# facebookresearch/goliath

Measured on AMD Instinct MI355X. Metric: relit views/sec (fwd+bwd) at 2048x1334, 250k Gaussians, higher is better.
Workload: dtype f32; 1 GPU; rgca_config2_envrelight; gaussians=250000, views_per_gpu=8, micro_batches=2, world_size=1, dist_backend=none, rccl_world_size=0, parallelism=view-parallel x1, launch=hip_graph_replay

## Files before the change

### goliath_amd/csrc/raster.hip

```cpp
#include <cstdlib>

#include "gol_raster.h"

namespace {

template <bool EXTRA, bool LAZY, int PPL>
__global__ __launch_bounds__(64 * Pix<PPL>::kWaves) void raster_fwd_kernel(
    int N, int img_h, int img_w, int planar, int tiles_x, int tiles_y, const int2* __restrict__ tile_bins,
    const int32_t* __restrict__ sorted_ids, int64_t capacity, const float* __restrict__ records,
    const float* __restrict__ background, float* __restrict__ out_img,
    float* __restrict__ out_extra, float* __restrict__ final_Ts, int32_t* __restrict__ final_idx,
    float* __restrict__ out_alpha, float* __restrict__ out_extra_norm, float norm_lo,
    const float* __restrict__ l1_target, const float* __restrict__ l1_mask, int l1_mask_c,
    uint8_t* __restrict__ l1_sign, float* __restrict__ l1_partial, int n_views) {
  typedef typename Pix<PPL>::fv fv;
  typedef typename Pix<PPL>::iv iv;
  constexpr int NW = Pix<PPL>::kWaves, NT = 64 * NW;
  __shared__ float s_l1[NW];
  __shared__ float4 s_a[kBatch];
  __shared__ float4 s_b[kBatch];
  __shared__ float2 s_c[kBatch];
  __shared__ int32_t s_mask[kBatch];
  const int T = tiles_x * tiles_y;
  const int view = blockIdx.x % n_views, slot = blockIdx.x / n_views;
  const TileCoord tc = tile_of_block(slot, T, tiles_x);
  if (!tc.ok) return;
  const int tid = threadIdx.x, lane = tid & 63, wave = tid >> 6;
  int j, i0;
  lane_pixel<PPL>(tc.tx, tc.ty, wave, lane, j, i0);
  bool in[PPL];
  fv py, live;
#pragma unroll
  for (int q = 0; q < PPL; ++q) {
    in[q] = (i0 + q < img_h) && (j < img_w);
    py[q] = (float)(i0 + q) + 0.5f;
    live[q] = in[q] ? 1.f : 0.f;
  }
  const float px = (float)j + 0.5f;

  const int2 range = tile_bins[(size_t)view * T + tc.tile];
  const int32_t* ids = sorted_ids + (size_t)view * capacity;
  const size_t goff = (size_t)view * N;

  fv T_cur = 1.f;
  iv cur_idx = 0;
  fv acc0 = 0.f, acc1 = 0.f, acc2 = 0.f, acc3 = 0.f;

  const int n_batches = (range.y - range.x + kBatch - 1) / kBatch;
  for (int bb = 0; bb < n_batches; ++bb) {
    if (__syncthreads_and(!any_live<fv, PPL>(live))) break;
    const int batch_start = range.x + bb * kBatch;
    for (int k = tid; k < kBatch; k += NT) {
      const int idx = batch_start + k;
      if (idx < range.y) {
        const Staged st = stage_entry<PPL>(records, goff + (size_t)ids[idx], (float)(tc.tx * 16), (float)(tc.ty * 16));
        s_a[k] = st.a; s_b[k] = st.b; s_c[k] = st.c; s_mask[k] = st.mask;
      } else {
        s_mask[k] = 0;
      }
    }
    __syncthreads();
    const int batch_size = min(kBatch, range.y - batch_start);
    for (int chunk = 0; chunk < batch_size; chunk += 64) {
      unsigned long long bits = gol_ballot((s_mask[chunk + lane] >> wave) & 1);
      if (LAZY && gol_ballot(any_live<fv, PPL>(live)) == 0ull) break;
      while (bits) {
        if (!LAZY && gol_ballot(any_live<fv, PPL>(live)) == 0ull) { chunk = batch_size; break; }
        const int t = chunk + __builtin_ctzll(bits);
        bits &= bits - 1;
        const float4 a4 = s_a[t];
        const float4 b4 = s_b[t];
        const float2 c2 = s_c[t];
        const float dx = a4.x - px;
        const fv dy = a4.y - py;
        fv sigma, e, alpha, vis, next_T;
        visit_falloff<PPL>(a4.z, a4.w, b4.x, dx, dy, sigma, e);
#pragma unroll
        for (int q = 0; q < PPL; ++q) alpha[q] = fminf(GOL_ALPHA_CAP_FWD, b4.y * e[q]);
        bool take[PPL];
        unsigned long long stop_m[PPL];
        const unsigned long long any_stop = fwd_step<PPL>(sigma, alpha, live, T_cur, vis, next_T, take, stop_m);
        bool half_done = false;
        if (!LAZY || any_stop != 0ull) {
#pragma unroll
          for (int q = 0; q < PPL; ++q) {
            const bool stop = __builtin_amdgcn_inverse_ballot_w64(stop_m[q]);
            live[q] = stop ? 0.f : live[q];
            if (LAZY) cur_idx[q] = stop ? (batch_start + t - 1) : cur_idx[q];
          }
          if (LAZY) half_done = gol_ballot(any_live<fv, PPL>(live)) == 0ull;
        }
        fwd_take<PPL>(take, next_T, vis, T_cur);
        acc0 += b4.z * vis; acc1 += b4.w * vis; acc2 += c2.x * vis;
        if (EXTRA) acc3 += c2.y * vis;
        if (!LAZY) {
#pragma unroll
          for (int q = 0; q < PPL; ++q) cur_idx[q] = take[q] ? (batch_start + t) : cur_idx[q];
        }
        if (LAZY && half_done) { chunk = batch_size; break; }
      }
    }
  }
  if (LAZY) {
#pragma unroll
    for (int q = 0; q < PPL; ++q) cur_idx[q] = live[q] != 0.f ? range.y - 1 : cur_idx[q];
  }

  const unsigned hw = (unsigned)img_h * (unsigned)img_w;
  const size_t vplane = (size_t)view * hw;
  float* __restrict__ o_T = final_Ts + vplane;
  int32_t* __restrict__ o_idx = final_idx + vplane;
  float* __restrict__ o_img = out_img + 3 * vplane;
  float* __restrict__ o_ex = (EXTRA && out_extra) ? out_extra + vplane : nullptr;
  float* __restrict__ o_alpha = out_alpha ? out_alpha + vplane : nullptr;
  float* __restrict__ o_norm = (EXTRA && out_extra_norm) ? out_extra_norm + vplane : nullptr;
  const float* __restrict__ i_tgt = l1_target ? l1_target + 3 * vplane : nullptr;
  const float* __restrict__ i_mask = l1_mask ? l1_mask + (size_t)l1_mask_c * vplane : nullptr;
  uint8_t* __restrict__ o_sign = l1_target ? l1_sign + vplane : nullptr;
  const float bg0 = background[0], bg1 = background[1], bg2 = background[2];
  float* __restrict__ o_img1 = o_img + (planar ? hw : 1u);
  float* __restrict__ o_img2 = o_img + (planar ? 2u * hw : 2u);
  const bool bwd_state = range.y > range.x;
  float l1_acc = 0.f;
#pragma unroll
  for (int q = 0; q < PPL; ++q) {
    if (!in[q]) continue;
    const unsigned pix = (unsigned)(i0 + q) * (unsigned)img_w + (unsigned)j;
    const unsigned b4 = pix * 4u;
    const unsigned bimg = planar ? b4 : 3u * b4;
    const float Tq = T_cur[q];
    const float c0 = acc0[q] + Tq * bg0, c1 = acc1[q] + Tq * bg1, c2 = acc2[q] + Tq * bg2, ex = acc3[q];
    *gol_at(o_T, b4) = Tq;
    if (bwd_state || !LAZY) *gol_at(o_idx, b4) = cur_idx[q];
    *gol_at(o_img, bimg) = c0; *gol_at(o_img1, bimg) = c1; *gol_at(o_img2, bimg) = c2;
    if (o_ex) *gol_at(o_ex, b4) = ex;
    if (o_alpha) *gol_at(o_alpha, b4) = 1.f - Tq;
    if (o_norm) *gol_at(o_norm, b4) = ex / fminf(fmaxf(1.f - Tq, norm_lo), 1.f);
    if (i_tgt) {
      const float m0 = i_mask ? *gol_at(i_mask, b4) : 1.f;
      const float cs[3] = {c0, c1, c2};
      unsigned code = 0u;
#pragma unroll
      for (int c = 0; c < 3; ++c) {
        const float m = (i_mask && l1_mask_c == 3) ? *gol_at(i_mask + (size_t)c * hw, b4) : m0;
        const float d = (cs[c] - *gol_at(i_tgt + (size_t)c * hw, b4)) * m;
        l1_acc += fabsf(d);
        code |= (d > 0.f ? 2u : (d < 0.f ? 0u : 1u)) << (2 * c);
      }
      if (bwd_state) *gol_at(o_sign, pix) = (uint8_t)code;
    }
  }
  if (l1_target) {
    const float ws = gol_wave_sum_to_lane63(l1_acc);
    if (lane == 63) s_l1[wave] = ws;
    __syncthreads();
    if (tid == 0) {
      float tot = 0.f;
#pragma unroll
      for (int w = 0; w < NW; ++w) tot += s_l1[w];
      l1_partial[(size_t)view * T + tc.tile] = tot;
    }
  }
}

__global__ __launch_bounds__(1024) void l1_sum_kernel(int n, const float* __restrict__ l1_partial, float scale,
                                                      float* __restrict__ l1_out) {
  __shared__ float s_w[16];
  float a0 = 0.f, a1 = 0.f, a2 = 0.f, a3 = 0.f;
  const int n4 = n >> 2;
  const float4* p4 = reinterpret_cast<const float4*>(l1_partial);
  int i = threadIdx.x;
  for (; i + 3 * 1024 < n4; i += 4 * 1024) {
    const float4 v0 = p4[i], v1 = p4[i + 1024], v2 = p4[i + 2048], v3 = p4[i + 3072];
    a0 += (v0.x + v0.y) + (v0.z + v0.w); a1 += (v1.x + v1.y) + (v1.z + v1.w);
    a2 += (v2.x + v2.y) + (v2.z + v2.w); a3 += (v3.x + v3.y) + (v3.z + v3.w);
  }
  for (; i < n4; i += 1024) { const float4 v = p4[i]; a0 += (v.x + v.y) + (v.z + v.w); }
  if ((int)threadIdx.x < (n & 3)) a1 += l1_partial[4 * n4 + threadIdx.x];
  const float ws = gol_wave_sum_to_lane63((a0 + a1) + (a2 + a3));
  if ((threadIdx.x & 63) == 63) s_w[threadIdx.x >> 6] = ws;
  __syncthreads();
  if (threadIdx.x == 0) {
    float tot = 0.f;
#pragma unroll
    for (int w = 0; w < 16; ++w) tot += s_w[w];
    l1_out[0] = tot * scale;
  }
}

constexpr int kBatchB = 64;
constexpr int kAcc = 12;

static_assert(kBatchB == 64, "raster_bwd_kernel ballots one 64-entry chunk per batch");

template <bool EXTRA, bool PACKED, int PPL>
__global__ __launch_bounds__(64 * Pix<PPL>::kWaves) void raster_bwd_kernel(
    int N, int img_h, int img_w, int planar, int tiles_x, int tiles_y, const int2* __restrict__ tile_bins,
    const int32_t* __restrict__ sorted_ids, int64_t capacity, const float* __restrict__ records,
    const float* __restrict__ background,
    const float* __restrict__ final_Ts, const int32_t* __restrict__ final_idx,
    const float* __restrict__ v_out_img, const float* __restrict__ v_out_extra,
    const float* __restrict__ v_out_alpha, float* __restrict__ v_xy, float* __restrict__ v_conic,
    float* __restrict__ v_colors, float* __restrict__ v_extra, float* __restrict__ v_opacity,
    const uint8_t* __restrict__ v_sign, const float* __restrict__ v_sign_mask, int v_sign_mask_c,
    const float* __restrict__ v_img_scale, float v_img_scale_mul, int n_views) {
  typedef typename Pix<PPL>::fv fv;
  typedef typename Pix<PPL>::iv iv;
  constexpr int NW = Pix<PPL>::kWaves, NT = 64 * NW;
  __shared__ StagedRow s_e[kBatchB];
  __shared__ int32_t s_mask[kBatchB];
  __shared__ int32_t s_id[kBatchB];
  __shared__ __attribute__((aligned(16))) float s_acc[NW][kBatchB][kAcc];
  __shared__ int32_t s_touched[NW][kBatchB];
  __shared__ int32_t s_wmax[NW];
  const int T = tiles_x * tiles_y;
  const int view = blockIdx.x % n_views, slot = blockIdx.x / n_views;
  const TileCoord tc = tile_of_block(slot, T, tiles_x);
  if (!tc.ok) return;
  const int2 range = tile_bins[(size_t)view * T + tc.tile];
  if (range.y <= range.x) return;
  const int tid = threadIdx.x, lane = tid & 63, wave = tid >> 6;
  int j, i0;
  lane_pixel<PPL>(tc.tx, tc.ty, wave, lane, j, i0);
  const float px = (float)j + 0.5f;
  const size_t hw = (size_t)img_h * img_w;
  const int32_t* ids = sorted_ids + (size_t)view * capacity;
  const size_t goff = (size_t)view * N;
  bool in[PPL];
  size_t pp[PPL];
  fv py, T_final;
  iv bin_final;
#pragma unroll
  for (int q = 0; q < PPL; ++q) {
    in[q] = (i0 + q < img_h) && (j < img_w);
    py[q] = (float)(i0 + q) + 0.5f;
    pp[q] = in[q] ? ((size_t)view * img_h + i0 + q) * img_w + j : 0;
    T_final[q] = in[q] ? final_Ts[pp[q]] : 1.f;
    bin_final[q] = in[q] ? final_idx[pp[q]] : (range.x - 1);
  }
  fv T_cur = T_final;
  fv vo0 = 0.f, vo1 = 0.f, vo2 = 0.f, vo3 = 0.f, voa = 0.f;
  {
    const float vsc = (v_img_scale ? v_img_scale[0] : 1.f) * v_img_scale_mul;
    const size_t os = planar ? hw : 1;
#pragma unroll
    for (int q = 0; q < PPL; ++q) {
      if (!in[q]) continue;
      const size_t p = pp[q];
      const int i = i0 + q;
      const size_t o = planar ? (size_t)view * 3 * hw + (size_t)i * img_w + j : 3 * p;
      float g0 = 0.f, g1 = 0.f, g2 = 0.f;
      if (v_out_img) { g0 = v_out_img[o]; g1 = v_out_img[o + os]; g2 = v_out_img[o + 2 * os]; }
      if (v_sign) {
        const unsigned code = v_sign[p];
        float m0 = vsc, m1 = vsc, m2 = vsc;
        if (v_sign_mask) {
          const float* mk = v_sign_mask + (size_t)view * v_sign_mask_c * hw + (size_t)i * img_w + j;
          m0 *= mk[0]; m1 *= (v_sign_mask_c == 3) ? mk[hw] : mk[0]; m2 *= (v_sign_mask_c == 3) ? mk[2 * hw] : mk[0];
        }
        g0 += (float)((int)(code & 3u) - 1) * m0;
        g1 += (float)((int)((code >> 2) & 3u) - 1) * m1;
        g2 += (float)((int)((code >> 4) & 3u) - 1) * m2;
      }
      vo0[q] = g0; vo1[q] = g1; vo2[q] = g2;
      if (EXTRA && v_out_extra) vo3[q] = v_out_extra[p];
      if (v_out_alpha) voa[q] = v_out_alpha[p];
    }
  }
  const fv tail = T_final * (voa - (background[0] * vo0 + background[1] * vo1 + background[2] * vo2));
  fv qsum = 0.f;

  const int wmax = wave_last_entry<PPL>(bin_final);
  if (lane == 0) s_wmax[wave] = wmax;
  __syncthreads();
  int bmax = s_wmax[0];
#pragma unroll
  for (int w = 1; w < NW; ++w) bmax = max(bmax, s_wmax[w]);
  bmax = min(bmax, range.y - 1);
  if (bmax < range.x) return;

  float* acc_lane = &s_acc[wave][0][lane >> 4];
  const int n_batches = (bmax - range.x + kBatchB) / kBatchB;
  auto entry_id = [&](int bb2) {
    const int e = bmax - bb2 * kBatchB - tid;
    return (tid < kBatchB && e >= range.x) ? ids[e] : 0;
  };
  int gid_next = entry_id(0);
  for (int bb = 0; bb < n_batches; ++bb) {
    __syncthreads();
    const int batch_end = bmax - bb * kBatchB;
    const int batch_size = min(kBatchB, batch_end + 1 - range.x);
    const int gid = gid_next;
    if (tid < kBatchB) {
      if (tid < batch_size) {
        const Staged st = stage_entry<PPL>(records, goff + (size_t)gid, (float)(tc.tx * 16), (float)(tc.ty * 16));
        s_e[tid].a = st.a; s_e[tid].b = st.b; s_e[tid].c = st.c; s_mask[tid] = st.mask;
        s_id[tid] = gid;
      } else {
        s_mask[tid] = 0;
      }
    }
    if (bb + 1 < n_batches) gid_next = entry_id(bb + 1);
    (&s_touched[0][0])[tid] = 0;
    __syncthreads();

    const int t0 = max(0, batch_end - wmax);
    unsigned long long bits = gol_ballot((s_mask[lane] >> wave) & 1);
    if (t0 > 0) bits &= ~0ull << t0;
    while (bits) {
      const int t = __builtin_ctzll(bits);
      bits &= bits - 1;
      const float4 a4 = s_e[t].a;
      const float4 b4 = s_e[t].b;
      const float2 c2 = s_e[t].c;
      const int li = batch_end - t;
      const float dx = a4.x - px;
      const fv dy = a4.y - py;
      fv sigma, vis, alpha, ra, fac;
      visit_falloff<PPL>(a4.z, a4.w, b4.x, dx, dy, sigma, vis);
      unsigned long long mv[PPL];
      if (bwd_taken<PPL>(b4.y, vis, sigma, li, bin_final, alpha, mv) == 0ull) continue;
      bool v[PPL];
      bwd_recur<PPL>(mv, alpha, T_cur, v, ra, fac);
      fv w = b4.z * vo0 + b4.w * vo1 + c2.x * vo2;
      if (EXTRA) w += c2.y * vo3;
      fv gop, gy, gyy;
      bwd_moments<PPL>(vis, w, T_cur, ra, fac, tail, v, dy, qsum, gop, gy, gyy);
      float g0s, g1s, g2s, g3 = 0.f;
      if (PPL == 2) {
        g0s = __builtin_fmaf(fac[0], vo0[0], fac[PPL - 1] * vo0[PPL - 1]);
        g1s = __builtin_fmaf(fac[0], vo1[0], fac[PPL - 1] * vo1[PPL - 1]);
        g2s = __builtin_fmaf(fac[0], vo2[0], fac[PPL - 1] * vo2[PPL - 1]);
        if (EXTRA) g3 = __builtin_fmaf(fac[0], vo3[0], fac[PPL - 1] * vo3[PPL - 1]);
      } else {
        g0s = fac[0] * vo0[0]; g1s = fac[0] * vo1[0]; g2s = fac[0] * vo2[0];
        if (EXTRA) g3 = fac[0] * vo3[0];
      }
      const float m0 = lane_sum<PPL>(gop), my = lane_sum<PPL>(gy), myy = lane_sum<PPL>(gyy);
      const float mx = m0 * dx, mxx = mx * dx, mxy = my * dx;
      const float r0 = gol_wave_sum4(g0s, g1s, g2s, m0);
      const float r1 = gol_wave_sum4(mx, my, mxx, mxy);
      const float r2 = gol_wave_sum_to_lane63(myy);
      const float r3 = EXTRA ? gol_wave_sum_to_lane63(g3) : 0.f;
      if ((lane & 15) == 15) {
        float* a = gol_at(acc_lane, (unsigned)t * (unsigned)(kAcc * sizeof(float)));
        a[0] = r0; a[4] = r1;
        if (lane == 63) { a[8 - 3] = r2; a[9 - 3] = r3; }
        s_touched[wave][t] = 1;
      }
    }
    __syncthreads();
    if (PACKED) {
      float* rec = v_colors;
      for (int idx = tid; idx < batch_size * 16; idx += NT) {
        const int t = idx >> 4, c = idx & 15;
        bool any = false;
#pragma unroll
        for (int w = 0; w < NW; ++w) any = any || (s_touched[w][t] != 0);
        if (!any || c > (EXTRA ? 9 : 8)) continue;
        const float4 a4 = s_e[t].a;
        const float4 b4 = s_e[t].b;
        const float nop = -b4.y, cc = b4.x;
        const int k1 = (c == 5) ? 4 : c, k2 = 5;
        const float w1 = (c == 4) ? nop * a4.z * kUnA : (c == 5) ? nop * a4.w * kUnB : (c == 6 || c == 8) ? 0.5f * nop
                       : (c == 7) ? nop : 1.f;
        const float w2 = (c == 4) ? nop * a4.w * kUnB : (c == 5) ? nop * cc * kUnA : 0.f;
        float s1 = 0.f, s2 = 0.f;
#pragma unroll
        for (int w = 0; w < NW; ++w) {
          const bool tw = s_touched[w][t] != 0;
          s1 += tw ? s_acc[w][t][k1] : 0.f;
          s2 += tw ? s_acc[w][t][k2] : 0.f;
        }
        atomicAdd(rec + (goff + (size_t)s_id[t]) * 16 + c, w1 * s1 + w2 * s2);
      }
    } else if (tid < batch_size) {
      float a[kAcc];
#pragma unroll
      for (int k = 0; k < kAcc; ++k) a[k] = 0.f;
      bool any = false;
#pragma unroll
      for (int w = 0; w < NW; ++w) {
        if (s_touched[w][tid]) {
          any = true;
          const float4* q = reinterpret_cast<const float4*>(&s_acc[w][tid][0]);
          const float4 q0 = q[0], q1 = q[1], q2 = q[2];
          a[0] += q0.x; a[1] += q0.y; a[2] += q0.z; a[3] += q0.w;
          a[4] += q1.x; a[5] += q1.y; a[6] += q1.z; a[7] += q1.w;
          a[8] += q2.x; a[9] += q2.y;
        }
      }
      if (any) {
        const size_t g = goff + (size_t)s_id[tid];
        const float4 a4 = s_e[tid].a;
        const float4 b4 = s_e[tid].b;
        const float nop = -b4.y;
        const float3 cn = true_conic(a4.z, a4.w, b4.x);
        atomicAdd(v_colors + 3 * g, a[0]); atomicAdd(v_colors + 3 * g + 1, a[1]); atomicAdd(v_colors + 3 * g + 2, a[2]);
        atomicAdd(v_opacity + g, a[3]);
        atomicAdd(v_xy + 2 * g, nop * (cn.x * a[4] + cn.y * a[5]));
        atomicAdd(v_xy + 2 * g + 1, nop * (cn.y * a[4] + cn.z * a[5]));
        atomicAdd(v_conic + 3 * g, 0.5f * nop * a[6]); atomicAdd(v_conic + 3 * g + 1, nop * a[7]);
        atomicAdd(v_conic + 3 * g + 2, 0.5f * nop * a[8]);
        if (EXTRA && v_extra) atomicAdd(v_extra + g, a[9]);
      }
    }
  }
}

__global__ __launch_bounds__(256) void raster_count_pairs_kernel(int N, int img_h, int img_w, int tiles_x, int tiles_y,
                                                                 const int2* __restrict__ tile_bins,
                                                                 const int32_t* __restrict__ sorted_ids, int64_t capacity,
                                                                 const float* __restrict__ records,
                                                                 const int32_t* __restrict__ final_idx,
                                                                 unsigned long long* __restrict__ counts) {
  __shared__ unsigned long long s_cnt[2];
  const int view = blockIdx.y, tile = blockIdx.x, T = tiles_x * tiles_y;
  const int ty = tile / tiles_x, tx = tile - ty * tiles_x;
  const int j = tx * 16 + (threadIdx.x & 15), i = ty * 16 + (threadIdx.x >> 4);
  if (threadIdx.x < 2) s_cnt[threadIdx.x] = 0ull;
  __syncthreads();
  const int2 range = tile_bins[(size_t)view * T + tile];
  unsigned long long tested = 0, taken = 0;
  if (i < img_h && j < img_w && range.y > range.x) {
    const int last = min(range.y - 1, final_idx[((size_t)view * img_h + i) * img_w + j]);
    const float px = (float)j + 0.5f, py = (float)i + 0.5f;
    for (int li = range.x; li <= last; ++li) {
      const float4* R = reinterpret_cast<const float4*>(records + ((size_t)view * N + sorted_ids[(size_t)view * capacity + li]) * GOL_SPLAT_RECORD);
      const float4 q0 = R[0], q1 = R[1];
      const float dx = q0.x - px, dy = q0.y - py;
      f1 sg, e;
      visit_falloff<1>(q0.z, q0.w, q1.x, dx, f1(dy), sg, e);
      const float alpha = fminf(GOL_ALPHA_CAP_FWD, q1.y * e[0]);
      ++tested;
      taken += (!(sg[0] < 0.f) && !(alpha < GOL_ALPHA_FLOOR)) ? 1 : 0;
    }
  }
  atomicAdd(&s_cnt[0], tested);
  atomicAdd(&s_cnt[1], taken);
  __syncthreads();
  if (threadIdx.x < 2 && s_cnt[threadIdx.x]) atomicAdd(counts + 2 * view + threadIdx.x, s_cnt[threadIdx.x]);
}

__global__ __launch_bounds__(256) void splat_pack_kernel(size_t n, const float* __restrict__ xys,
                                                         const float* __restrict__ conics,
                                                         const float* __restrict__ colors,
                                                         const float* __restrict__ extra,
                                                         const float* __restrict__ opacities,
                                                         float* __restrict__ records) {
  const size_t e = (size_t)blockIdx.x * 256 + threadIdx.x;
  if (e >= n) return;
  gol_record_write(records + e * GOL_SPLAT_RECORD, xys[2 * e], xys[2 * e + 1], conics[3 * e], conics[3 * e + 1],
                   conics[3 * e + 2], opacities[e], colors ? colors[3 * e] : 0.f, colors ? colors[3 * e + 1] : 0.f,
                   colors ? colors[3 * e + 2] : 0.f, extra ? extra[e] : 0.f);
}

}

extern "C" int gol_raster_plan(int B, int* fwd_pixels_per_lane) {
  static const int forced = getenv("GOL_RASTER_PPL") ? atoi(getenv("GOL_RASTER_PPL")) : 0;
  if (fwd_pixels_per_lane) *fwd_pixels_per_lane = (forced == 1 || forced == 2) ? forced : (B <= 2 ? 1 : 2);
  return GOL_OK;
}

extern "C" int gol_raster_count_pairs(int B, int N, int img_h, int img_w, const int32_t* tile_bins, const int32_t* sorted_ids,
                                      int64_t capacity, const float* records, const int32_t* final_idx, uint64_t* counts,
                                      void* stream) {
  GOL_REQUIRE(B >= 0 && N >= 0 && img_h > 0 && img_w > 0, "bad size");
  if (B == 0) return GOL_OK;
  GOL_REQUIRE(tile_bins && final_idx && counts && (capacity == 0 || sorted_ids) && (N == 0 || records), "null pointer");
  hipStream_t s = (hipStream_t)stream;
  if (hipMemsetAsync(counts, 0, sizeof(uint64_t) * 2 * (size_t)B, s) != hipSuccess) {
    gol_set_error("gol_raster_count_pairs: hipMemsetAsync failed");
    return GOL_ERR_LAUNCH;
  }
  const int tiles_x = (img_w + 15) / 16, tiles_y = (img_h + 15) / 16;
  raster_count_pairs_kernel<<<dim3(tiles_x * tiles_y, B), 256, 0, s>>>(
      N, img_h, img_w, tiles_x, tiles_y, reinterpret_cast<const int2*>(tile_bins), sorted_ids, capacity, records, final_idx,
      reinterpret_cast<unsigned long long*>(counts));
  GOL_CHECK_LAUNCH();
  return GOL_OK;
}

extern "C" int gol_splat_pack(int B, int N, const float* xys, const float* conics, const float* colors,
                              const float* extra, const float* opacities, float* records, void* stream) {
  GOL_REQUIRE(B >= 0 && N >= 0, "negative size");
  if (B == 0 || N == 0) return GOL_OK;
  GOL_REQUIRE(xys && conics && opacities && records, "null pointer");
  const size_t n = (size_t)B * N;
  splat_pack_kernel<<<gol_cdiv((long long)n, 256), 256, 0, (hipStream_t)stream>>>(n, xys, conics, colors, extra, opacities,
                                                                                 records);
  GOL_CHECK_LAUNCH();
  return GOL_OK;
}

extern "C" int gol_rasterize_fwd(int B, int N, int img_h, int img_w, int block, int planar, const int32_t* tile_bins,
                                 const int32_t* sorted_ids, int64_t capacity, const float* records, int with_extra,
                                 const float* background, float* out_img,
                                 float* out_extra, float* final_Ts, int32_t* final_idx, float* out_alpha,
                                 float* out_extra_norm, float norm_lo, const float* l1_target, const float* l1_mask,
                                 int l1_mask_c, uint8_t* l1_sign, float* l1_partial, float* l1_out, float l1_scale,
                                 int pixels_per_lane, void* stream) {
  GOL_RASTER_CHECK_DIMS(12, "image too large (32-bit byte offsets inside a view)");
  if (B == 0) return GOL_OK;
  GOL_REQUIRE(tile_bins && background && out_img && final_Ts && final_idx, "null pointer");
  GOL_REQUIRE(capacity == 0 || sorted_ids, "null sorted_ids");
  GOL_REQUIRE(N == 0 || records, "null Gaussian records");
  GOL_REQUIRE((!out_extra && !out_extra_norm) || with_extra || N == 0, "out_extra / out_extra_norm need the extra channel");
  GOL_REQUIRE(!with_extra || out_extra || out_extra_norm, "extra without an output for it");
  GOL_REQUIRE(!l1_target || (planar && l1_sign && l1_partial), "the fused L1 needs planar images, l1_sign and l1_partial");
  GOL_REQUIRE(!l1_mask || (l1_target && (l1_mask_c == 1 || l1_mask_c == 3)), "l1_mask: 1 or 3 channels, with l1_target");
  GOL_REQUIRE(!l1_out || l1_target, "l1_out needs l1_target");
  const int tiles_x = (img_w + 15) / 16, tiles_y = (img_h + 15) / 16;
  const dim3 grid((unsigned)raster_grid(B, img_h, img_w));
  const int2* bins = reinterpret_cast<const int2*>(tile_bins);
  hipStream_t s = (hipStream_t)stream;
  GOL_REQUIRE(pixels_per_lane >= 0 && pixels_per_lane <= 2, "pixels_per_lane: 0 (choose by B), 1 or 2");
  int ppl = pixels_per_lane;
  if (ppl == 0) gol_raster_plan(B, &ppl);
  auto launch = [&](auto ex_c, auto lazy_c) {
    with_ppl(ppl, [&](auto ppl_c) {
      constexpr bool EX = decltype(ex_c)::value, LZ = decltype(lazy_c)::value;
      constexpr int PPL = decltype(ppl_c)::value;
      raster_fwd_kernel<EX, LZ, PPL><<<grid, 64 * Pix<PPL>::kWaves, 0, s>>>(
          N, img_h, img_w, planar, tiles_x, tiles_y, bins, sorted_ids, capacity, records, background, out_img, out_extra,
          final_Ts, final_idx, out_alpha, EX ? out_extra_norm : nullptr, norm_lo, l1_target, l1_mask, l1_mask_c, l1_sign,
          l1_partial, B);
    });
  };
  const bool ex = out_extra || out_extra_norm;
  if (ex && planar) launch(kYes, kYes);
  else if (ex) launch(kYes, kNo);
  else if (planar) launch(kNo, kYes);
  else launch(kNo, kNo);
  if (l1_out) l1_sum_kernel<<<1, 1024, 0, s>>>(B * tiles_x * tiles_y, l1_partial, l1_scale, l1_out);
  GOL_CHECK_LAUNCH();
  return GOL_OK;
}

extern "C" int gol_rasterize_bwd(int B, int N, int img_h, int img_w, int block, int planar, const int32_t* tile_bins,
                                 const int32_t* sorted_ids, int64_t capacity, const float* records, int with_extra,
                                 const float* background, const float* final_Ts,
                                 const int32_t* final_idx, const float* v_out_img, const float* v_out_extra,
                                 const float* v_out_alpha, float* v_xy, float* v_conic, float* v_colors,
                                 float* v_extra, float* v_opacity, int grad_stride, const uint8_t* v_sign,
                                 const float* v_sign_mask, int v_sign_mask_c, const float* v_img_scale,
                                 float v_img_scale_mul, int pixels_per_lane, void* stream) {
  GOL_RASTER_CHECK_DIMS(0, "");
  if (B == 0 || N == 0 || capacity == 0) return GOL_OK;
  GOL_REQUIRE(tile_bins && sorted_ids && background && final_Ts && final_idx, "null pointer");
  GOL_REQUIRE(v_out_img || v_sign, "no upstream image gradient (v_out_img or v_sign)");
  GOL_REQUIRE(!v_sign || planar, "the sign image of the fused L1 goes with planar images");
  GOL_REQUIRE(!v_sign_mask || (v_sign && (v_sign_mask_c == 1 || v_sign_mask_c == 3)), "v_sign_mask: 1 or 3 channels, with v_sign");
  GOL_REQUIRE(records, "null Gaussian records");
  GOL_REQUIRE(v_xy && v_conic && v_colors && v_opacity, "null gradient output");
  GOL_REQUIRE(!(v_out_extra || v_extra) || with_extra, "extra-channel gradients need the extra channel");
  GOL_REQUIRE(grad_stride == 0 || grad_stride == GOL_GRAD_RECORD, "grad_stride must be 0 (dense arrays) or 16 (records)");
  const bool packed = grad_stride == GOL_GRAD_RECORD;
  if (packed)
    GOL_REQUIRE(v_opacity == v_colors + 3 && v_xy == v_colors + 4 && v_conic == v_colors + 6 &&
                    (!v_extra || v_extra == v_colors + 9),
                "record layout is [rgb | opacity | xy | conic | extra | pad] (GOL_GRAD_RECORD floats)");
  const int tiles_x = (img_w + 15) / 16, tiles_y = (img_h + 15) / 16;
  const dim3 grid((unsigned)raster_grid(B, img_h, img_w));
  const int2* bins = reinterpret_cast<const int2*>(tile_bins);
  hipStream_t s = (hipStream_t)stream;
  GOL_REQUIRE(pixels_per_lane >= 0 && pixels_per_lane <= 2, "pixels_per_lane: 0 (2), 1 or 2");
  const int ppl = pixels_per_lane ? pixels_per_lane : 2;
  const bool ex = with_extra && (v_out_extra || v_extra);
  auto launch = [&](auto ex_c, auto packed_c) {
    with_ppl(ppl, [&](auto ppl_c) {
      constexpr bool EX = decltype(ex_c)::value, PK = decltype(packed_c)::value;
      constexpr int PPL = decltype(ppl_c)::value;
      raster_bwd_kernel<EX, PK, PPL><<<grid, 64 * Pix<PPL>::kWaves, 0, s>>>(
          N, img_h, img_w, planar, tiles_x, tiles_y, bins, sorted_ids, capacity, records, background, final_Ts, final_idx,
          v_out_img, EX ? v_out_extra : nullptr, v_out_alpha, v_xy, v_conic, v_colors, EX ? v_extra : nullptr, v_opacity,
          v_sign, v_sign_mask, v_sign_mask_c, v_img_scale, v_img_scale_mul, B);
    });
  };
  if (ex && packed) launch(kYes, kYes);
  else if (ex) launch(kYes, kNo);
  else if (packed) launch(kNo, kYes);
  else launch(kNo, kNo);
  GOL_CHECK_LAUNCH();
  return GOL_OK;
}
```

Baseline: 2973 views/s.

## Pre-reduce packed gradient partials per entry before chunked atomic flush

In the packed backward path, each entry's per-wave accumulators are now summed once by one thread, and the gradient weights are applied there. The finished record is written back into wave-0 shared slots, replacing a per-(entry,channel) loop that redid the wave reduction and weight selection for every channel. After a barrier, lanes map to channels and issue the atomics in unrolled chunks of four entries, with the record stride held in a scalar register. This adds an extra barrier and shared-memory traffic, and it relies on stale flags in s_touched[0] being cleared for entries beyond batch_size.

```diff
diff --git a/goliath_amd/csrc/raster.hip b/goliath_amd/csrc/raster.hip
--- a/goliath_amd/csrc/raster.hip
+++ b/goliath_amd/csrc/raster.hip
@@ -286,6 +286,8 @@
     return (tid < kBatchB && e >= range.x) ? ids[e] : 0;
   };
   int gid_next = entry_id(0);
+  unsigned rec_bytes = GOL_GRAD_RECORD * sizeof(float);
+  if (PACKED) asm volatile("" : "+s"(rec_bytes));
   for (int bb = 0; bb < n_batches; ++bb) {
     __syncthreads();
     const int batch_end = bmax - bb * kBatchB;
@@ -351,28 +353,60 @@
     }
     __syncthreads();
     if (PACKED) {
-      float* rec = v_colors;
-      for (int idx = tid; idx < batch_size * 16; idx += NT) {
-        const int t = idx >> 4, c = idx & 15;
+      if (tid < kBatchB) {
+        int tw[NW];
+#pragma unroll
+        for (int w = 0; w < NW; ++w) tw[w] = s_touched[w][tid];
+        float s[kAcc];
+#pragma unroll
+        for (int k = 0; k < kAcc; ++k) s[k] = 0.f;
         bool any = false;
 #pragma unroll
-        for (int w = 0; w < NW; ++w) any = any || (s_touched[w][t] != 0);
-        if (!any || c > (EXTRA ? 9 : 8)) continue;
-        const float4 a4 = s_e[t].a;
-        const float4 b4 = s_e[t].b;
-        const float nop = -b4.y, cc = b4.x;
-        const int k1 = (c == 5) ? 4 : c, k2 = 5;
-        const float w1 = (c == 4) ? nop * a4.z * kUnA : (c == 5) ? nop * a4.w * kUnB : (c == 6 || c == 8) ? 0.5f * nop
-                       : (c == 7) ? nop : 1.f;
-        const float w2 = (c == 4) ? nop * a4.w * kUnB : (c == 5) ? nop * cc * kUnA : 0.f;
-        float s1 = 0.f, s2 = 0.f;
-#pragma unroll
         for (int w = 0; w < NW; ++w) {
-          const bool tw = s_touched[w][t] != 0;
-          s1 += tw ? s_acc[w][t][k1] : 0.f;
-          s2 += tw ? s_acc[w][t][k2] : 0.f;
+          if (tw[w]) {
+            any = true;
+            const float4* q = reinterpret_cast<const float4*>(&s_acc[w][tid][0]);
+            const float4 q0 = q[0], q1 = q[1], q2 = q[2];
+            s[0] += q0.x; s[1] += q0.y; s[2] += q0.z; s[3] += q0.w;
+            s[4] += q1.x; s[5] += q1.y; s[6] += q1.z; s[7] += q1.w;
+            s[8] += q2.x; s[9] += q2.y;
+          }
         }
-        atomicAdd(rec + (goff + (size_t)s_id[t]) * 16 + c, w1 * s1 + w2 * s2);
+        if (any) {
+          const float4 a4 = s_e[tid].a;
+          const float4 b4 = s_e[tid].b;
+          const float nop = -b4.y, cc = b4.x;
+          const float wxx = nop * a4.z * kUnA, wxy = nop * a4.w * kUnB, wyy = nop * cc * kUnA, hnop = 0.5f * nop;
+          float4* o = reinterpret_cast<float4*>(&s_acc[0][tid][0]);
+          o[0] = make_float4(s[0], s[1], s[2], s[3]);
+          o[1] = make_float4(wxx * s[4] + wxy * s[5], wxy * s[4] + wyy * s[5], hnop * s[6], nop * s[7]);
+          *reinterpret_cast<float2*>(o + 2) = make_float2(hnop * s[8], s[9]);
+          s_touched[0][tid] = 1;
+        }
+      }
+      __syncthreads();
+      const int c = tid & 15;
+      if (c <= (EXTRA ? 9 : 8)) {
+        float* rec_c = v_colors + goff * 16 + c;
+        constexpr int kIt = kBatchB * 16 / NT, kCh = 4;
+        static_assert(kIt % kCh == 0, "the merge issues its atomics in chunks of kCh entries per lane");
+#pragma unroll
+        for (int i0 = 0; i0 < kIt; i0 += kCh) {
+          int flag[kCh], id[kCh];
+          float val[kCh];
+#pragma unroll
+          for (int i = 0; i < kCh; ++i) {
+            const int t = (tid >> 4) + (i0 + i) * (NT / 16);
+            flag[i] = s_touched[0][t]; id[i] = s_id[t]; val[i] = s_acc[0][t][c];
+          }
+#pragma unroll
+          for (int i = 0; i < kCh; ++i) {
+            if (flag[i]) {
+              char* r = reinterpret_cast<char*>(rec_c) + (uint64_t)(unsigned)id[i] * rec_bytes;
+              atomicAdd(reinterpret_cast<float*>(r), val[i]);
+            }
+          }
+        }
       }
     } else if (tid < batch_size) {
       float a[kAcc];
```

Result: faster. 3040 views/s, median of 6 (+2.3%).
